# soham97/mellow

Hardware: AMD Instinct MI355X
Metric: audio-pair responses/sec (v0 167M, 2x10s clips, max_len=64, greedy) (higher is better)
Workload: dtype f32 (encoder/prefill GEMM operands split EXACTLY into 3 bf16 terms, 6 bf16 MFMA products per fp32 product, f32 accumulate: fp32-accurate, parity suite green; mel included, the STFT is an fp32 FFT; attentions and decode on exact fp32 MFMA / VALU)

## Files before the change

mellow_amd/csrc/encoder.hip:

```cpp
#include <cstdlib>

#include "common.h"
#include "kernels.h"

namespace mellow {

__global__ void reflect_pad_kernel(const float* __restrict__ wav, int64_t n, float* __restrict__ out, int64_t plen,
                                   int pad) {
    const int c = blockIdx.y;
    const float* src = wav + (int64_t)c * n;
    float* dst = out + (int64_t)c * plen;
    for (int64_t i = (int64_t)blockIdx.x * blockDim.x + threadIdx.x; i < plen; i += (int64_t)gridDim.x * blockDim.x) {
        int64_t j = i - pad;
        if (j < 0) j = -j;
        if (j >= n) j = 2 * (n - 1) - j;
        if (j < 0) j = 0;
        if (j >= n) j = n - 1;
        dst[i] = src[j];
    }
}
void launch_reflect_pad(const float* wav, int n_clips, int64_t n_samples, float* out, int64_t padded_len, int pad,
                        hipStream_t s) {
    hipLaunchKernelGGL(reflect_pad_kernel, dim3(512, n_clips), dim3(256), 0, s, wav, n_samples, out, padded_len, pad);
}
// ... 403 lines not shown
    }
}
void launch_rmsnorm_apb(const float* in, void* out_apb, int M, int C, const float* w, float eps, hipStream_t s, void* out_scales) {
    const size_t lds = (size_t)32 * (C + 4) * sizeof(float);
    set_max_dynamic_lds(reinterpret_cast<const void*>(&rmsnorm_apb_kernel<false>), 96 * 1024);
    set_max_dynamic_lds(reinterpret_cast<const void*>(&rmsnorm_apb_kernel<true>), 96 * 1024);
    if (out_scales) hipLaunchKernelGGL(rmsnorm_apb_kernel<true>, dim3((M + 31) / 32), dim3(256), lds, s, in, reinterpret_cast<i32x4*>(out_apb), (int64_t)M, C, w, eps, reinterpret_cast<uint8_t*>(out_scales));
    else hipLaunchKernelGGL(rmsnorm_apb_kernel<false>, dim3((M + 31) / 32), dim3(256), lds, s, in, reinterpret_cast<i32x4*>(out_apb), (int64_t)M, C, w, eps, (uint8_t*)nullptr);
}
void launch_rmsnorm(const float* in, float* out, int M, int C, const float* w, float eps, hipStream_t s) {
    hipLaunchKernelGGL(rmsnorm_kernel, dim3((M + 3) / 4), dim3(256), 0, s, in, out, (int64_t)M, C, w, eps);
}

__device__ __forceinline__ void wa_ld4(const float* base, int64_t elem, bool in16, float (&o)[4]) {
    if (in16) {
        typedef unsigned u32x2_ __attribute__((ext_vector_type(2)));
        const u32x2_ r = *reinterpret_cast<const u32x2_*>(reinterpret_cast<const uint16_t*>(base) + elem);
        o[0] = __uint_as_float(r[0] << 16); o[1] = __uint_as_float(r[0] & 0xffff0000u); o[2] = __uint_as_float(r[1] << 16); o[3] = __uint_as_float(r[1] & 0xffff0000u);
    } else {
        const float4 r = *reinterpret_cast<const float4*>(base + elem);
        o[0] = r.x; o[1] = r.y; o[2] = r.z; o[3] = r.w;
    }
}
template <bool IN16>
__global__ __launch_bounds__(256) void window_attention_mfma_kernel(const float* __restrict__ qkv, float* __restrict__ out,
                                                                    int C, int nH, const float* __restrict__ bias_exp,
                                                                    const float* __restrict__ mask, int nW,
                                                                    int64_t n_tiles, i32x4* __restrict__ out_apb) {
    __shared__ __attribute__((aligned(16))) float Vs[4][64 * 24];
    const int lane = threadIdx.x & 63, wave = threadIdx.x >> 6;
    const int64_t tile = (int64_t)blockIdx.x * 4 + wave;
    const bool active = tile < n_tiles;
    const int64_t win = active ? tile / nH : 0;
    const int hd = active ? (int)(tile % nH) : 0;
    const int h = lane >> 5, ml = lane & 31;
    const float scale = 0.20412414523193150818f;
    float kf[2][12], qf[2][12];
#pragma unroll
    for (int t = 0; t < 2; ++t) {
        const int64_t row = (win * 64 + t * 32 + ml) * (3 * C) + hd * 24 + 12 * h;
#pragma unroll
        for (int v = 0; v < 3; ++v) {
            float q4[4], k4[4];
            wa_ld4(qkv, row + v * 4, IN16, q4);
            wa_ld4(qkv, row + C + v * 4, IN16, k4);
#pragma unroll
            for (int j = 0; j < 4; ++j) { qf[t][4 * v + j] = q4[j] * scale; kf[t][4 * v + j] = k4[j]; }
        }
    }
    {
        const int64_t vrow = (win * 64 + lane) * (3 * C) + 2 * C + hd * 24;
#pragma unroll
        for (int v = 0; v < 6; ++v) {
            float v4[4];
            wa_ld4(qkv, vrow + v * 4, IN16, v4);
            *reinterpret_cast<float4*>(&Vs[wave][lane * 24 + v * 4]) = make_float4(v4[0], v4[1], v4[2], v4[3]);
        }
    }
    f32x16 S[2][2];
#pragma unroll
    for (int kt = 0; kt < 2; ++kt)
#pragma unroll
        for (int qt = 0; qt < 2; ++qt) {
#pragma unroll
            for (int r = 0; r < 16; ++r) S[kt][qt][r] = 0.f;
#pragma unroll
            for (int s_ = 0; s_ < 12; ++s_) S[kt][qt] = __builtin_amdgcn_mfma_f32_32x32x2f32(kf[kt][s_], qf[qt][s_], S[kt][qt], 0, 0, 0);
        }
    float inv[2];
#pragma unroll
    for (int qt = 0; qt < 2; ++qt) {
        const int qi = qt * 32 + ml;
        const float* brow = bias_exp + ((int64_t)hd * 64 + qi) * 64;
        const float* mrow = mask ? mask + ((win % nW) * 64 + qi) * 64 : nullptr;
        float mx = -INFINITY;
#pragma unroll
        for (int kt = 0; kt < 2; ++kt)
#pragma unroll
            for (int g4 = 0; g4 < 4; ++g4) {
                const int k0 = kt * 32 + 8 * g4 + 4 * h;
                const float4 b4 = *reinterpret_cast<const float4*>(brow + k0);
                float add[4] = {b4.x, b4.y, b4.z, b4.w};
                if (mrow) {
                    const float4 m4 = *reinterpret_cast<const float4*>(mrow + k0);
                    S[kt][qt][4 * g4 + 0] = (S[kt][qt][4 * g4 + 0] + add[0]) + m4.x;
                    S[kt][qt][4 * g4 + 1] = (S[kt][qt][4 * g4 + 1] + add[1]) + m4.y;
                    S[kt][qt][4 * g4 + 2] = (S[kt][qt][4 * g4 + 2] + add[2]) + m4.z;
                    S[kt][qt][4 * g4 + 3] = (S[kt][qt][4 * g4 + 3] + add[3]) + m4.w;
                } else {
#pragma unroll
                    for (int j = 0; j < 4; ++j) S[kt][qt][4 * g4 + j] += add[j];
                }
#pragma unroll
                for (int j = 0; j < 4; ++j) mx = fmaxf(mx, S[kt][qt][4 * g4 + j]);
            }
        mx = half_max(mx);
        float sum = 0.f;
#pragma unroll
        for (int kt = 0; kt < 2; ++kt)
#pragma unroll
            for (int r = 0; r < 16; ++r) {
                const float pv = __builtin_amdgcn_exp2f((S[kt][qt][r] - mx) * 1.44269504088896340736f);
                S[kt][qt][r] = pv;
                sum += pv;
            }
        inv[qt] = 1.0f / half_sum(sum);
    }
    __syncthreads();
    f32x16 O[2];
#pragma unroll
    for (int qt = 0; qt < 2; ++qt)
#pragma unroll
        for (int r = 0; r < 16; ++r) O[qt][r] = 0.f;
    const float* Vc = Vs[wave];
#pragma unroll
    for (int kt = 0; kt < 2; ++kt)
#pragma unroll
        for (int r = 0; r < 16; ++r) {
            const int key = kt * 32 + (r & 3) + 8 * (r >> 2) + 4 * h;
            const float a = ml < 24 ? Vc[key * 24 + ml] : 0.f;
            O[0] = __builtin_amdgcn_mfma_f32_32x32x2f32(a, S[kt][0][r], O[0], 0, 0, 0);
            O[1] = __builtin_amdgcn_mfma_f32_32x32x2f32(a, S[kt][1][r], O[1], 0, 0, 0);
        }
    if (active && out_apb) {
        const int KT = C >> 4;
#pragma unroll
        for (int qt = 0; qt < 2; ++qt) {
            const int64_t m = win * 64 + qt * 32 + ml;
            float X[4], Y[4], Z[4], w[8];
#pragma unroll
            for (int j = 0; j < 4; ++j) { X[j] = O[qt][j] * inv[qt]; Y[j] = O[qt][4 + j] * inv[qt]; Z[j] = O[qt][8 + j] * inv[qt]; }
            apb_store_quads(out_apb, m, hd * 3, KT, X, Y, h);
#pragma unroll
            for (int j = 0; j < 4; ++j) {
                auto r = __builtin_amdgcn_permlane32_swap(__float_as_uint(Z[j]), __float_as_uint(Z[j]), false, false);
                w[j] = __uint_as_float(r[0]);
                w[4 + j] = __uint_as_float(r[1]);
            }
            if (h == 0) apb_store8(out_apb, m, hd * 3 + 2, KT, w);
        }
    } else if (active) {
#pragma unroll
        for (int qt = 0; qt < 2; ++qt) {
            float* dst = out + (win * 64 + qt * 32 + ml) * C + hd * 24;
#pragma unroll
            for (int g4 = 0; g4 < 3; ++g4) {
                const int d = 8 * g4 + 4 * h;
                *reinterpret_cast<float4*>(dst + d) = make_float4(O[qt][4 * g4] * inv[qt], O[qt][4 * g4 + 1] * inv[qt],
                                                                  O[qt][4 * g4 + 2] * inv[qt], O[qt][4 * g4 + 3] * inv[qt]);
            }
        }
    }
}
void launch_window_attention(const float* qkv, float* out, int M, int C, int nH, const float* bias_exp,
                             const float* mask, int nW, hipStream_t s, void* out_apb, bool qkv16) {
    const int64_t n_tiles = (int64_t)(M / 64) * nH;
    if (qkv16) {
        hipLaunchKernelGGL(window_attention_mfma_kernel<true>, dim3((unsigned)((n_tiles + 3) / 4)), dim3(256), 0, s, qkv, out, C, nH,
                           bias_exp, mask, nW, n_tiles, reinterpret_cast<i32x4*>(out_apb));
        return;
    }
    hipLaunchKernelGGL(window_attention_mfma_kernel<false>, dim3((unsigned)((n_tiles + 3) / 4)), dim3(256), 0, s, qkv, out, C, nH,
                       bias_exp, mask, nW, n_tiles, reinterpret_cast<i32x4*>(out_apb));
}

__global__ __launch_bounds__(256) void tail_latent_im2col_kernel(const float* __restrict__ y, float* __restrict__ latent,
                                                                 int64_t latent_stride, float* __restrict__ a_ts) {
    const int clip = blockIdx.x;
    const float* yc = y + (int64_t)clip * 64 * 768;
    for (int ch = threadIdx.x; ch < 768; ch += 256) {
        float sacc = 0.f;
        for (int cf = 0; cf < 2; ++cf)
            for (int tt = 0; tt < 32; ++tt) {
                const int tok = ((tt >> 3) * 2 + cf) * 8 + (tt & 7);
                sacc += yc[tok * 768 + ch];
            }
        latent[(int64_t)clip * latent_stride + ch] = sacc * (1.0f / 64.0f);
    }
    float4* dst = reinterpret_cast<float4*>(a_ts + (int64_t)clip * 32 * 4608);
    for (int i = threadIdx.x; i < 32 * 6 * 192; i += 256) {
        const int c4 = i % 192;
        const int seg = (i / 192) % 6;
        const int tt = i / (192 * 6);
        const int cf = seg / 3, dt = seg % 3;
        const int ts = tt + dt - 1;
        float4 v = make_float4(0.f, 0.f, 0.f, 0.f);
// ... 179 lines not shown
```

mellow_amd/csrc/engine.cpp:

```cpp
#include "engine_internal.h"

static thread_local std::string g_err;
int fail(const char* fmt, ...) {
    char buf[1024];
    va_list ap;
    va_start(ap, fmt);
    vsnprintf(buf, sizeof(buf), fmt, ap);
    va_end(ap);
    g_err = buf;
    return 1;
}
int ensure(mellow_engine* e, mellow_engine::Buf& b, size_t floats) {
    if (b.cap >= floats) return 0;
    if (b.p) HIPCHK(hipFree(b.p));
    b.p = nullptr;
    b.cap = 0;
    HIPCHK(hipMalloc(&b.p, floats * sizeof(float)));
    b.cap = floats;
    return 0;
}
int dev_alloc(mellow_engine* e, float** out, size_t floats) {
    const size_t bytes = (floats * sizeof(float) + 4095) / 4096 * 4096;
    if (!e->arena) {
        const size_t want = (size_t)(e->opt.arena_mb < 0 ? 0 : e->opt.arena_mb) << 20;
// ... 310 lines not shown
            HIPCHK(hipStreamCreateWithFlags(&st, hipStreamNonBlocking));
            int rc = streams_overlap(e, e->stream, st, &ok);
            for (int k = 1; k < h && ok && !rc; ++k) rc = streams_overlap(e, e->stream2[k - 1], st, &ok);
            if (rc) { hipStreamDestroy(st); return rc; }
            if (ok) e->stream2[h - 1] = st; else hipStreamDestroy(st);
        }
        if (!ok) {
            e->prefill_parts_want = e->prefill_parts;
            e->prefill_parts = e->prefill_parts_ok = h;
            e->streams_probed = true;
            break;
        }
    }
    return 0;
}
struct OptDesc { const char* key; const char* dflt; bool answers; const char* what; };
static const OptDesc kOptions[] = {
    {"prefill_split", "2", false, "f32x3: parts of the split LM prefill (1..4); bit-identical for every value"},
    {"prefill_fuse_norm", "1", true, "f32x3: norm-free LM prefill (GEMM epilogues emit split output + RMS partials); 0 = a normalisation launch per GEMM input"},
    {"decode_fuse", "1", true, "down projection of layer l fused with q/k/v of layer l + 1 through the load-time product W'Wd; 0 = five launches per layer"},
    {"decode_fuse_max_rb", "1", true, "largest number of 32-row blocks that runs the fused down + q/k/v launch on fp32 weights"},
    {"splitk", "8", true, "f32x3 encoder: largest split count of the split-K launches (0 = never split; a summation order)"},
    {"enc_apb", "0x1CC", false, "f32x3 encoder: Swin stages whose producers hand over pre-split (bit st, 4 + st, 8 + st); bit-identical"},
    {"graph", "1", false, "decode steps as hipGraph replays (0 = eager launches)"},
    {"fp8_decode", "1", true, "fp8 mode: e4m3 weights in the decode kernels"},
    {"fp8_prefill", "1", true, "fp8 mode: e4m3 GEMMs in encoder + LM prefill"},
    {"fp8_decode_act", "1", true, "fp8 mode: e4m3 activations in the decode GEMM kernels (fp8 matrix pipe)"},
    {"fp8_kv16", "1", true, "fp8 mode: bf16 shadow of the K/V pages for the decode step"},
    {"fp8_attn_bf16", "1", true, "fp8 mode: q / k / v stored once as bf16 (LM: bf16 K/V pages + bf16-once prefill attention; Swin: bf16 q/k/v rows into the exact window attention); 0 = fp32 q/k/v, the 3-way split attention"},
    {"decode_x3", "7", true, "f32x3: mask of decode GEMM launches on the bf16 pipe (1 lm_head, 2 gate/up, 4 fused down + q/k/v)"},
    {"decode_x3_min_rb", "2", true, "f32x3: fewest 32-row blocks at which the layer launches take their f32x3 forms"},
    {"x3_stft", "1", true, "f32x3: STFT / mel GEMMs on the split kernel (0 = exact fp32 kernel)"},
    {"stft_fft", "1", true, "f32x3: STFT as a 1024-point FFT when the checkpoint's conv weights are the windowed DFT basis"},
    {"x3_apb", "1", true, "f32x3 LM prefill: producers hand over pre-split, GEMMs staged by LDS-DMA (0 = register-staged kernel on fp32 activations)"},
    {"x3_attn", "1", true, "f32x3: prefill attention on exact bf16 splits (0 = exact fp32 MFMA kernel)"},
    {"x3w", "1", false, "f32x3: K = 96 GEMMs on the weight-stationary persistent kernel; bit-identical"},
    {"row_migration", "1", false, "reference-semantics loop, B > 32: rows still running are packed into the lowest 32-row blocks; tokens unchanged"},
    {"arena_mb", "3400", false, "size of the weight arena in MiB (before the first tensor is loaded)"},
};
static const OptDesc* find_opt(const char* key) {
    for (const auto& o : kOptions)
        if (!strcmp(o.key, key)) return &o;
    return nullptr;
}
static long opt_val(const mellow_engine* e, const char* key) {
    auto it = e->opt.given.find(key);
    return strtol(it != e->opt.given.end() ? it->second.c_str() : find_opt(key)->dflt, nullptr, 0);
}
int apply_options(mellow_engine* e) {
    const int mode = e->opt.mode;
    e->prefill_parts = (int)opt_val(e, "prefill_split");
    e->opt.prefill_fuse_norm = opt_val(e, "prefill_fuse_norm") != 0;
    e->opt.decode_fuse = opt_val(e, "decode_fuse") != 0;
    e->opt.dec_fuse_max_rb = (int)opt_val(e, "decode_fuse_max_rb");
    e->opt.sk_max = (int)opt_val(e, "splitk");
    e->opt.enc_apb_stages = (int)opt_val(e, "enc_apb");
    e->use_graph = opt_val(e, "graph") != 0;
    e->opt.x3_stft = opt_val(e, "x3_stft") != 0;
    e->opt.stft_fft = opt_val(e, "stft_fft") != 0 && e->opt.x3_stft;
    e->opt.x3_apb = opt_val(e, "x3_apb") != 0;
    e->opt.x3_attn = opt_val(e, "x3_attn") != 0;
    e->opt.x3w = opt_val(e, "x3w") != 0;
    e->opt.row_migration = opt_val(e, "row_migration") != 0;
    e->opt.arena_mb = (int)opt_val(e, "arena_mb");
    e->opt.fp8 = mode == MELLOW_PRECISION_FP8;
    e->opt.fp8_decode = e->opt.fp8 && opt_val(e, "fp8_decode") != 0;
    e->opt.fp8_decode_act = e->opt.fp8_decode && opt_val(e, "fp8_decode_act") != 0;
    e->opt.fp8_prefill = opt_val(e, "fp8_prefill") != 0;
    e->opt.fp8_attn_bf16 = opt_val(e, "fp8_attn_bf16") != 0;
    e->opt.kv16 = e->opt.fp8_decode && opt_val(e, "fp8_kv16") != 0;
    e->opt.f32x3_terms = mode == MELLOW_PRECISION_F32X3 ? 6 : 0;
    e->opt.dec_x3 = mode == MELLOW_PRECISION_F32X3 ? ((int)opt_val(e, "decode_x3") & DEC_X3_ALL) : 0;
    e->opt.dec_x3_min_rb = (int)opt_val(e, "decode_x3_min_rb") < 1 ? 1 : (int)opt_val(e, "decode_x3_min_rb");
    return 0;
}

extern "C" {

int mellow_engine_set_option(mellow_engine_t* e, const char* key, const char* value) {
// ... 135 lines not shown
```

mellow_amd/csrc/engine_encoder.cpp:

```cpp
#include "engine_internal.h"

static void with_splitk(mellow_engine* e, GemmArgs& g) {
    if (!e->sk_enable || e->opt.sk_max < 2 || !e->sk_ws.p) return;
    g.sk_ws = e->sk_ws.p;
    g.sk_tiles = 256;
    g.sk_max = e->opt.sk_max;
}
int run_gemm(mellow_engine* e, const GemmArgs& a) {
    const bool x3_stft = e->opt.x3_stft;
    if (e->opt.f32x3_terms && a.K % 16 == 0 &&
        ((a.a_mode == A_PLAIN && (a.epi == EPI_LINEAR || a.epi == EPI_SWIGLU || a.epi == EPI_QKV_ROPE || a.epi == EPI_QKV_ROPE_AT)) || (x3_stft && a.K >= 192))) {
        auto it = e->w.bf_w.find(a.Wp);
        if (it != e->w.bf_w.end()) {
            GemmArgs g = a;
            g.W8 = reinterpret_cast<const uint8_t*>(it->second);
            with_splitk(e, g);
            ProfScope ps(e, PF_GEMM, gemm_flops(a), 0.0);
            ps.r.M = a.M; ps.r.N = a.Nw; ps.r.K = a.K; ps.r.epi = a.epi + 200;
            launch_gemm_bf16x3_fused(g, e->stream);
            return 0;
        }
    }
    if (e->opt.fp8 && e->opt.fp8_prefill && a.a_mode == A_PLAIN && (a.epi == EPI_LINEAR || a.epi == EPI_SWIGLU || a.epi == EPI_QKV_ROPE)) {
        auto it = e->w.fp8_w.find(a.Wp);
// ... 104 lines not shown
    CHK(ensure(e, e->QKV, (size_t)M0 * 288));
    CHK(ensure(e, e->H, (size_t)M0 * 384));
    {
        ProfScope ps(e, PF_MISC, 0, (double)M0 * 96 * 4);
        launch_fold_patch_embed(e->logmel.p, n, frames, n_crops, crop_hop, crop_len, e->w.pe_w, e->w.pe_b, e->w.pe_nw, e->w.pe_nb,
                                e->X0.p, s);
    }
    CHK(tap(e, "patch", e->X0.p, M0 * 96));
    float *x = e->X0.p, *x2 = e->X1.p, *t = e->T.p;
    for (int st = 0; st < 4; ++st) {
        const int C = 96 << st, R = 64 >> st, N = R * R, nH = kHeads[st];
        const int nW = R > kWin ? (R / kWin) * (R / kWin) : 1;
        const int M1 = nv * N;
        for (int b = 0; b < kDepths[st]; ++b) {
            const SwinBlockW& w = e->w.blocks[st][b];
            const bool shifted = (b % 2 == 1) && R > kWin;
            const int32_t* map = R > kWin ? e->w.win_map[st][shifted ? 1 : 0] : nullptr;
            const bool amx = e->opt.fp8 && e->opt.fp8_prefill && e->opt.x3_apb && e->w.fp8_w.count(w.qkv.p) && e->w.fp8_w.count(w.fc1.p) && e->w.fp8_w.count(w.fc2.p);
            const bool have_pb = e->opt.f32x3_terms && e->w.bf_w.count(w.qkv.p) && e->w.bf_w.count(w.fc1.p) && e->w.bf_w.count(w.fc2.p);
            const bool apb_h = amx || (have_pb && ((e->opt.enc_apb_stages >> st) & 1));
            const bool apb = apb_h || (have_pb && ((e->opt.enc_apb_stages >> (8 + st)) & 1));
            const size_t M1p = (size_t)rup(M1, 128);
            char *a3s = nullptr, *h3s = nullptr;
            if (apb) {
                CHK(ensure(e, e->enc_a3, (M1p * C * 6 + 3) / 4));
                if (apb_h) CHK(ensure(e, e->enc_h3, (M1p * 4 * C * 6 + 3) / 4));
                if (amx) {
                    a3s = reinterpret_cast<char*>(e->enc_a3.p) + M1p * rup(C, 64);
                    h3s = reinterpret_cast<char*>(e->enc_h3.p) + M1p * rup(4 * C, 64);
                }
                { ProfScope ps(e, PF_NORM, 0, 2.5 * M1 * C * 4); launch_layernorm_apb(x, e->enc_a3.p, M1, C, w.n1w, w.n1b, map, N, s, a3s); }
                {
                    GemmArgs g = lin(nullptr, C, M1, w.qkv, e->QKV.p, 3 * C, w.qkv_b);
                    g.c16 = (amx && e->opt.fp8_attn_bf16) ? 1 : 0;
                    CHK(run_gemm_apb(e, g, e->enc_a3.p, s, a3s));
                }
            } else {
                { ProfScope ps(e, PF_NORM, 0, 2.0 * M1 * C * 4); launch_layernorm(x, t, M1, C, w.n1w, w.n1b, map, N, s); }
                CHK(run_gemm(e, lin(t, C, M1, w.qkv, e->QKV.p, 3 * C, w.qkv_b)));
            }
            const bool apb_proj = apb && !amx && ((e->opt.enc_apb_stages >> (4 + st)) & 1) && e->w.bf_w.count(w.proj.p);
            {
                ProfScope ps(e, PF_WINDOW_ATTN, 4.0 * 64 * 64 * 24 * (double)(M1 / 64) * nH, 4.0 * M1 * C * 4);
                launch_window_attention(e->QKV.p, t, M1, C, nH, w.bias_exp, shifted ? w.mask : nullptr, nW, s, apb_proj ? e->enc_a3.p : nullptr, amx && e->opt.fp8_attn_bf16);
            }
            {
                GemmArgs g = lin(t, C, M1, w.proj, x, C, w.proj_b);
                g.resid = x; g.ldr = C; g.crow_map = map; g.rows_in = N; g.rows_out = N;
                if (apb_proj) CHK(run_gemm_apb(e, g, e->enc_a3.p, s));
                else CHK(run_gemm(e, g));
            }
            if (apb) {
                { ProfScope ps(e, PF_NORM, 0, 2.5 * M1 * C * 4); launch_layernorm_apb(x, e->enc_a3.p, M1, C, w.n2w, w.n2b, nullptr, N, s, a3s); }
                {
                    GemmArgs g = lin(nullptr, C, M1, w.fc1, apb_h ? nullptr : e->H.p, 4 * C, w.fc1_b);
                    g.act = ACT_GELU; g.C3 = apb_h ? e->enc_h3.p : nullptr;
                    if (amx) { g.c3_fmt = 1; g.C3s = reinterpret_cast<uint8_t*>(h3s); g.c3_kt64 = rup(4 * C, 64) / 64; }
                    CHK(run_gemm_apb(e, g, e->enc_a3.p, s, a3s));
                }
                {
                    GemmArgs g = lin(apb_h ? nullptr : e->H.p, 4 * C, M1, w.fc2, x, C, w.fc2_b);
                    g.resid = x; g.ldr = C;
                    if (apb_h) CHK(run_gemm_apb(e, g, e->enc_h3.p, s, h3s));
                    else CHK(run_gemm(e, g));
                }
            } else {
                { ProfScope ps(e, PF_NORM, 0, 2.0 * M1 * C * 4); launch_layernorm(x, t, M1, C, w.n2w, w.n2b, nullptr, N, s); }
                {
                    GemmArgs g = lin(t, C, M1, w.fc1, e->H.p, 4 * C, w.fc1_b);
                    g.act = ACT_GELU;
                    CHK(run_gemm(e, g));
                }
// ... 167 lines not shown
```

mellow_amd/csrc/engine_internal.h:

```cpp
#pragma once
#include <hip/hip_runtime.h>

#include <array>
#include <chrono>
#include <cmath>
#include <cstdarg>
#include <cstdio>
#include <cstdlib>
#include <cstring>
#include <map>
#include <unordered_map>
#include <string>
#include <thread>
#include <type_traits>
#include <utility>
#include <vector>

#include "../../include/mellow_hip.h"
#include "kernels.h"

using namespace mellow;

int fail(const char* fmt, ...);
struct mellow_engine;
// ... 30 lines not shown
    std::vector<char> data;
    std::vector<int64_t> shape;
    int dtype = 0;
    int64_t numel() const {
        int64_t n = 1;
        for (auto d : shape) n *= d;
        return n;
    }
    const float* f() const { return reinterpret_cast<const float*>(data.data()); }
};

struct Packed {
    float* p = nullptr;
    int N = 0, K = 0, NP = 0, KP = 0;
    int Nw = 0;
};

struct SwinBlockW {
    float *n1w, *n1b, *n2w, *n2b;
    Packed qkv, proj, fc1, fc2;
    float *qkv_b, *proj_b, *fc1_b, *fc2_b;
    float* bias_exp;
    float* mask;
};
struct MergeW {
    float *nw, *nb;
    Packed red;
};
struct DecW {
    const float *p, *scale;
};
struct LMLayerW {
    Packed qkv, o, gateup, down;
    Packed qkv_f, gateup_f;
    float* o16 = nullptr;
    float* gu16n = nullptr;
    float* gu16 = nullptr;
    float* qkv2 = nullptr;
    float *q2h8 = nullptr, *q2h_sc = nullptr;
    float *qkv8 = nullptr, *qkv_sc = nullptr, *o8 = nullptr, *o_sc = nullptr, *gu8 = nullptr, *gu_sc = nullptr, *dn8 = nullptr,
          *dn_sc = nullptr;
    float *in_ln, *post_ln;
    DecW qkv_w() const { return qkv8 ? DecW{qkv8, qkv_sc} : DecW{qkv_f.p, nullptr}; }
    DecW o_w() const { return o8 ? DecW{o8, o_sc} : DecW{o16, nullptr}; }
    DecW gateup_w() const { return gu8 ? DecW{gu8, gu_sc} : DecW{gu16, nullptr}; }
    DecW down_w() const { return dn8 ? DecW{dn8, dn_sc} : DecW{down.p, nullptr}; }
// ... 45 lines not shown
        float* p = nullptr;
        size_t cap = 0;
        Buf() = default; Buf(const Buf&) = delete; Buf& operator=(const Buf&) = delete;
        Buf(Buf&& o) noexcept : p(o.p), cap(o.cap) { o.p = nullptr; o.cap = 0; }
        Buf& operator=(Buf&& o) noexcept { std::swap(p, o.p); std::swap(cap, o.cap); return *this; }
        LOCAL ~Buf() { if (p) (void)hipFree(p); }
    };
    struct LOCAL Options {
        std::map<std::string, std::string> given;
        int mode = MELLOW_PRECISION_F32X3;
        bool x3_stft = true, stft_fft = true, x3_apb = true, x3_attn = true, x3w = true, row_migration = true, decode_fuse = true;
        int arena_mb = 3400;
        bool kv16 = false;
        bool fp8 = false;
        bool fp8_decode = false;
        bool fp8_decode_act = false;
        bool fp8_attn_bf16 = true;
        bool fp8_prefill = true;
        int dec_x3_min_rb = 2;
        int dec_x3 = 0;
        int f32x3_terms = 0;
        bool prefill_fuse_norm = true;
        int enc_apb_stages = 0x1CC;
        int sk_max = 8;
        int dec_fuse_max_rb = 1;
    };
    struct Fp8W { uint8_t* w8; float* scale; };
    struct LOCAL Weights {
        Packed dft, mel;
        float *fft_win = nullptr, *fft_tw1 = nullptr, *fft_tw2 = nullptr;
        float *bn_alpha = nullptr, *bn_beta = nullptr;
        float *pe_w = nullptr, *pe_b = nullptr, *pe_nw = nullptr, *pe_nb = nullptr;
        std::vector<SwinBlockW> blocks[4];
        MergeW merge[3];
        int32_t* win_map[4][2] = {{nullptr}};
        float *fn_w = nullptr, *fn_b = nullptr;
        Packed tscam, c2l, lin1, lin2;
        float *tscam_b = nullptr, *c2l_b = nullptr, *pln_w = nullptr, *pln_b = nullptr;
        int32_t* emb_row_map = nullptr;
        float* embed = nullptr;
        Packed lm_head;
        std::vector<LMLayerW> layers;
        float* final_norm = nullptr;
        float *rope_cos = nullptr, *rope_sin = nullptr;
        float *head8 = nullptr, *head_sc = nullptr;
        DecW head_w() const { return head8 ? DecW{head8, head_sc} : DecW{lm_head.p, nullptr}; }
// ... 206 lines not shown
```

mellow_amd/csrc/engine_weights.cpp:

```cpp
#include "engine_internal.h"

static const HostTensor* get(mellow_engine* e, const std::string& k) {
    auto it = e->host.find(k);
    return it == e->host.end() ? nullptr : &it->second;
}
static int expect_shape(const HostTensor* t, const std::string& k, std::initializer_list<int64_t> shp) {
    if (!t) return fail("missing key in state_dict: %s", k.c_str());
    if (t->dtype != MELLOW_F32) return fail("%s: expected float32", k.c_str());
    if (t->shape.size() != shp.size())
        return fail("size mismatch for %s: rank %d in the checkpoint, %d expected", k.c_str(), (int)t->shape.size(), (int)shp.size());
    size_t i = 0;
    for (auto d : shp) {
        if (t->shape[i] != d)
            return fail("size mismatch for %s: dimension %d is %lld in the checkpoint, %lld expected", k.c_str(), (int)i,
                        (long long)t->shape[i], (long long)d);
        ++i;
    }
    return 0;
}
static int up_vec(mellow_engine* e, const std::string& k, int64_t n, float** out, int64_t pad_to = 0) {
    const HostTensor* t = get(e, k);
    CHK(expect_shape(t, k, {n}));
    return upload(e, out, t->f(), (size_t)n, (size_t)pad_to);
}
// ... 151 lines not shown
        CHK(upload(e, &e->w.pe_w, get(e, k)->f(), 96 * 16));
        CHK(up_vec(e, E + "patch_embed.proj.bias", 96, &e->w.pe_b));
        CHK(up_vec(e, E + "patch_embed.norm.weight", 96, &e->w.pe_nw));
        CHK(up_vec(e, E + "patch_embed.norm.bias", 96, &e->w.pe_nb));
    }
    for (int s = 0; s < 4; ++s) {
        const int C = 96 << s, nH = kHeads[s], R = 64 >> s, nW = (R / kWin) * (R / kWin);
        for (int sh = 0; sh < 2; ++sh) {
            if (R <= kWin) continue;
            std::vector<int32_t> m((size_t)R * R);
            window_map_host(R, sh ? kWin / 2 : 0, m.data());
            float* d = nullptr;
            CHK(upload(e, &d, reinterpret_cast<const float*>(m.data()), m.size()));
            e->w.win_map[s][sh] = reinterpret_cast<int32_t*>(d);
        }
        for (int b = 0; b < kDepths[s]; ++b) {
            const std::string p = E + "layers." + std::to_string(s) + ".blocks." + std::to_string(b) + ".";
            SwinBlockW w{};
            CHK(up_vec(e, p + "norm1.weight", C, &w.n1w));
            CHK(up_vec(e, p + "norm1.bias", C, &w.n1b));
            CHK(up_vec(e, p + "norm2.weight", C, &w.n2w));
            CHK(up_vec(e, p + "norm2.bias", C, &w.n2b));
            CHK(pack_key(e, p + "attn.qkv.weight", 3 * C, C, &w.qkv));
            CHK(pack_key(e, p + "attn.proj.weight", C, C, &w.proj));
            CHK(pack_key(e, p + "mlp.fc1.weight", 4 * C, C, &w.fc1));
            CHK(pack_key(e, p + "mlp.fc2.weight", C, 4 * C, &w.fc2));
            CHK(up_vec(e, p + "attn.qkv.bias", 3 * C, &w.qkv_b, w.qkv.NP));
            CHK(up_vec(e, p + "attn.proj.bias", C, &w.proj_b, w.proj.NP));
            CHK(up_vec(e, p + "mlp.fc1.bias", 4 * C, &w.fc1_b, w.fc1.NP));
            CHK(up_vec(e, p + "mlp.fc2.bias", C, &w.fc2_b, w.fc2.NP));
            const HostTensor *tb = get(e, p + "attn.relative_position_bias_table"), *ix = get(e, p + "attn.relative_position_index");
            CHK(expect_shape(tb, p + "attn.relative_position_bias_table", {225, nH}));
            if (ix->numel() != 64 * 64) return fail("size mismatch for %sattn.relative_position_index", p.c_str());
            std::vector<float> be((size_t)nH * 4096);
            for (int i = 0; i < 4096; ++i) {
                int64_t id;
                if (ix->dtype == MELLOW_I64) id = reinterpret_cast<const int64_t*>(ix->data.data())[i];
                else id = reinterpret_cast<const int32_t*>(ix->data.data())[i];
                if (id < 0 || id >= 225) return fail("relative_position_index out of range");
                for (int h = 0; h < nH; ++h) be[(size_t)h * 4096 + i] = tb->f()[id * nH + h];
            }
            CHK(upload(e, &w.bias_exp, be.data(), be.size()));
            w.mask = nullptr;
            if ((b % 2 == 1) && R > kWin) {
                const std::string km = p + "attn_mask";
                CHK(expect_shape(get(e, km), km, {nW, 64, 64}));
// ... 160 lines not shown
```

mellow_amd/csrc/kernels.h:

```cpp
#pragma once
#include <hip/hip_runtime.h>
#include <stdint.h>

namespace mellow {

void launch_pack_weight(const float* w, int N, int K, int64_t ldw, float* out, int NP, int KP, hipStream_t s);
void launch_pack_weight_pairs(const float* w0, const float* w1, int N, int K, int64_t ldw, float* out, int NP,
                              int KP, hipStream_t s);

enum { ACT_NONE = 0, ACT_GELU = 1, ACT_SIGMOID = 2 };
enum { EPI_LINEAR = 0, EPI_POWER = 1, EPI_LOGMEL = 2, EPI_SWIGLU = 3, EPI_QKV_ROPE = 4, EPI_LSE = 5, EPI_QKV_ROPE_AT = 6 };
enum { A_PLAIN = 0, A_FRAMES = 1 };

struct GemmArgs {
    const float* A = nullptr;
    int64_t lda = 0;
    int M = 0;
    int K = 0;
    int a_mode = A_PLAIN;
    int fpc = 1;
    int64_t clip_stride = 0;
    int hop = 0;
    const float* Wp = nullptr;
    int Nw = 0;
// ... 242 lines not shown
void set_gemm_debug_buffer(uint64_t* p);

void launch_resample(const float* x, int n_clips, int64_t n_in, const float* wT, int orig, int nw, int klen, int width,
                     float* out, int64_t n_out, hipStream_t s);
void launch_reflect_pad(const float* wav, int n_clips, int64_t n_samples, float* out, int64_t padded_len, int pad,
                        hipStream_t s);
void launch_fold_patch_embed(const float* logmel_bn, int n_src, int src_frames, int n_crops, int crop_hop,
                             int crop_len, const float* conv_w, const float* conv_b, const float* ln_w,
                             const float* ln_b, float* x0, hipStream_t s);

void launch_layernorm(const float* in, float* out, int M, int C, const float* w, const float* b,
                      const int32_t* row_map, int ntok, hipStream_t s);
void launch_merge_layernorm(const float* in, float* out, int n, int R, int C, const float* w, const float* b,
                            hipStream_t s);
void launch_stft_fft_power(const float* wpad, int fpc, int64_t clip_stride, int hop, int M, const float* win, const float* tw1,
                           const float* tw2, float* power, hipStream_t s);
void launch_rmsnorm(const float* in, float* out, int M, int C, const float* w, float eps, hipStream_t s);
void launch_layernorm_apb(const float* in, void* out_apb, int M, int C, const float* w, const float* b, const int32_t* row_map,
                          int ntok, hipStream_t s, void* out_scales = nullptr);
void launch_rmsnorm_apb(const float* in, void* out_apb, int M, int C, const float* w, float eps, hipStream_t s, void* out_scales = nullptr);

void launch_window_attention(const float* qkv, float* out, int M, int C, int nH, const float* bias_exp,
                             const float* mask, int nW, hipStream_t s, void* out_apb = nullptr, bool qkv16 = false);

void launch_tail_latent_im2col(const float* y, int n, float* latent, int64_t latent_stride, float* a_ts,
                               hipStream_t s);
void launch_crop_average(const float* in, int n, int n_crops, int64_t len, int64_t in_stride, float* out,
                         int64_t out_stride, hipStream_t s);
void launch_gelu(const float* in, float* out, int64_t n, hipStream_t s);
void launch_prefix_assemble(const float* proj33, const float* embed, const int32_t* ids, int B, int text_len,
                            int sep_id, int vocab, float* prefix, unsigned long long* bad_id_word, hipStream_t s);
void launch_prefix_assemble_q(const float* proj33, const float* embed, const int32_t* ids, int B, int Q, int text_len, int P,
                              int sep_id, int vocab, float* head, float* tail, unsigned long long* bad_id_word, hipStream_t s);
void launch_gather_rows(const float* table, int width, const int32_t* ids, int n, int n_rows, float* out, hipStream_t s);
void launch_gather_span(const float* in, int B, int T, int from_pos, int n, float* out, hipStream_t s);
void launch_clear_page_slots(float* cache, int64_t pages, int Tmax, int t0, int t1, hipStream_t s, bool pages16 = false);
void launch_downsample33(const float* proj33, int n, float* out, hipStream_t s);

void launch_prefill_attention(const float* q, const float* k_cache, const float* v_cache, float* o, void* o_apb, int B, int T,
                              int Tmax, bool x3, hipStream_t s, void* o_scales = nullptr, bool bf16_once = false, bool pages16 = false);
void launch_prefill_attention_past(const float* q, const float* k_cache, const float* v_cache, float* o, void* o_apb, int B, int T,
                                   int Tmax, int q0, bool x3, hipStream_t s);
void launch_lse_merge(const float2* part_ms, const int32_t* part_arg, int64_t ld, int groups, int rows, const int32_t* targets,
                      const float* tgt_logit, int vocab, float* out_logprob, int32_t* out_argmax, float* out_lse, float* out_max,
                      unsigned long long* bad_word, hipStream_t s);
void launch_score_build_input(const float* prefix, const float* embed, const int32_t* cand_ids, const int32_t* cand_len, int K,
// ... 7 lines not shown
```

Before: 459.6.

## Fuse Swin qkv GEMM with window attention for early encoder stages

Adds a kernel that computes the per-head q/k/v projection with split-bf16 MFMA for each 64-token window and feeds the result straight into the existing window attention tile. This avoids writing and re-reading the full QKV tensor for stages 0 (enabled by default via a bitmask option). Per-head weights are pre-packed at load time and staged in LDS. The cost is a persistent-style grid with heavier register and LDS use per workgroup, which may reduce occupancy compared with the separate GEMM.

```diff
diff --git a/mellow_amd/csrc/encoder.hip b/mellow_amd/csrc/encoder.hip
--- a/mellow_amd/csrc/encoder.hip
+++ b/mellow_amd/csrc/encoder.hip
@@ -449,6 +449,105 @@
         o[0] = r.x; o[1] = r.y; o[2] = r.z; o[3] = r.w;
     }
 }
+__device__ __forceinline__ void window_attention_tile(const float (&kf)[2][12], const float (&qf)[2][12], const float* Vc, float* __restrict__ out,
+                                                      int C, int64_t win, int hd, bool active, const float* __restrict__ bias_exp,
+                                                      const float* __restrict__ mask, int nW, i32x4* __restrict__ out_apb) {
+    const int lane = threadIdx.x & 63;
+    const int h = lane >> 5, ml = lane & 31;
+    f32x16 S[2][2];
+#pragma unroll
+    for (int kt = 0; kt < 2; ++kt)
+#pragma unroll
+        for (int qt = 0; qt < 2; ++qt) {
+#pragma unroll
+            for (int r = 0; r < 16; ++r) S[kt][qt][r] = 0.f;
+#pragma unroll
+            for (int s_ = 0; s_ < 12; ++s_) S[kt][qt] = __builtin_amdgcn_mfma_f32_32x32x2f32(kf[kt][s_], qf[qt][s_], S[kt][qt], 0, 0, 0);
+        }
+    float inv[2];
+#pragma unroll
+    for (int qt = 0; qt < 2; ++qt) {
+        const int qi = qt * 32 + ml;
+        const float* brow = bias_exp + ((int64_t)hd * 64 + qi) * 64;
+        const float* mrow = mask ? mask + ((win % nW) * 64 + qi) * 64 : nullptr;
+        float mx = -INFINITY;
+#pragma unroll
+        for (int kt = 0; kt < 2; ++kt)
+#pragma unroll
+            for (int g4 = 0; g4 < 4; ++g4) {
+                const int k0 = kt * 32 + 8 * g4 + 4 * h;
+                const float4 b4 = *reinterpret_cast<const float4*>(brow + k0);
+                float add[4] = {b4.x, b4.y, b4.z, b4.w};
+                if (mrow) {
+                    const float4 m4 = *reinterpret_cast<const float4*>(mrow + k0);
+                    S[kt][qt][4 * g4 + 0] = (S[kt][qt][4 * g4 + 0] + add[0]) + m4.x;
+                    S[kt][qt][4 * g4 + 1] = (S[kt][qt][4 * g4 + 1] + add[1]) + m4.y;
+                    S[kt][qt][4 * g4 + 2] = (S[kt][qt][4 * g4 + 2] + add[2]) + m4.z;
+                    S[kt][qt][4 * g4 + 3] = (S[kt][qt][4 * g4 + 3] + add[3]) + m4.w;
+                } else {
+#pragma unroll
+                    for (int j = 0; j < 4; ++j) S[kt][qt][4 * g4 + j] += add[j];
+                }
+#pragma unroll
+                for (int j = 0; j < 4; ++j) mx = fmaxf(mx, S[kt][qt][4 * g4 + j]);
+            }
+        mx = half_max(mx);
+        float sum = 0.f;
+#pragma unroll
+        for (int kt = 0; kt < 2; ++kt)
+#pragma unroll
+            for (int r = 0; r < 16; ++r) {
+                const float pv = __builtin_amdgcn_exp2f((S[kt][qt][r] - mx) * 1.44269504088896340736f);
+                S[kt][qt][r] = pv;
+                sum += pv;
+            }
+        inv[qt] = 1.0f / half_sum(sum);
+    }
+    __syncthreads();
+    f32x16 O[2];
+#pragma unroll
+    for (int qt = 0; qt < 2; ++qt)
+#pragma unroll
+        for (int r = 0; r < 16; ++r) O[qt][r] = 0.f;
+#pragma unroll
+    for (int kt = 0; kt < 2; ++kt)
+#pragma unroll
+        for (int r = 0; r < 16; ++r) {
+            const int key = kt * 32 + (r & 3) + 8 * (r >> 2) + 4 * h;
+            const float a = ml < 24 ? Vc[key * 24 + ml] : 0.f;
+            O[0] = __builtin_amdgcn_mfma_f32_32x32x2f32(a, S[kt][0][r], O[0], 0, 0, 0);
+            O[1] = __builtin_amdgcn_mfma_f32_32x32x2f32(a, S[kt][1][r], O[1], 0, 0, 0);
+        }
+    if (active && out_apb) {
+        const int KT = C >> 4;
+#pragma unroll
+        for (int qt = 0; qt < 2; ++qt) {
+            const int64_t m = win * 64 + qt * 32 + ml;
+            float X[4], Y[4], Z[4], w[8];
+#pragma unroll
+            for (int j = 0; j < 4; ++j) { X[j] = O[qt][j] * inv[qt]; Y[j] = O[qt][4 + j] * inv[qt]; Z[j] = O[qt][8 + j] * inv[qt]; }
+            apb_store_quads(out_apb, m, hd * 3, KT, X, Y, h);
+#pragma unroll
+            for (int j = 0; j < 4; ++j) {
+                auto r = __builtin_amdgcn_permlane32_swap(__float_as_uint(Z[j]), __float_as_uint(Z[j]), false, false);
+                w[j] = __uint_as_float(r[0]);
+                w[4 + j] = __uint_as_float(r[1]);
+            }
+            if (h == 0) apb_store8(out_apb, m, hd * 3 + 2, KT, w);
+        }
+    } else if (active) {
+#pragma unroll
+        for (int qt = 0; qt < 2; ++qt) {
+            float* dst = out + (win * 64 + qt * 32 + ml) * C + hd * 24;
+#pragma unroll
+            for (int g4 = 0; g4 < 3; ++g4) {
+                const int d = 8 * g4 + 4 * h;
+                *reinterpret_cast<float4*>(dst + d) = make_float4(O[qt][4 * g4] * inv[qt], O[qt][4 * g4 + 1] * inv[qt],
+                                                                  O[qt][4 * g4 + 2] * inv[qt], O[qt][4 * g4 + 3] * inv[qt]);
+            }
+        }
+    }
+}
 template <bool IN16>
 __global__ __launch_bounds__(256) void window_attention_mfma_kernel(const float* __restrict__ qkv, float* __restrict__ out,
                                                                     int C, int nH, const float* __restrict__ bias_exp,
@@ -484,100 +583,7 @@
             *reinterpret_cast<float4*>(&Vs[wave][lane * 24 + v * 4]) = make_float4(v4[0], v4[1], v4[2], v4[3]);
         }
     }
-    f32x16 S[2][2];
-#pragma unroll
-    for (int kt = 0; kt < 2; ++kt)
-#pragma unroll
-        for (int qt = 0; qt < 2; ++qt) {
-#pragma unroll
-            for (int r = 0; r < 16; ++r) S[kt][qt][r] = 0.f;
-#pragma unroll
-            for (int s_ = 0; s_ < 12; ++s_) S[kt][qt] = __builtin_amdgcn_mfma_f32_32x32x2f32(kf[kt][s_], qf[qt][s_], S[kt][qt], 0, 0, 0);
-        }
-    float inv[2];
-#pragma unroll
-    for (int qt = 0; qt < 2; ++qt) {
-        const int qi = qt * 32 + ml;
-        const float* brow = bias_exp + ((int64_t)hd * 64 + qi) * 64;
-        const float* mrow = mask ? mask + ((win % nW) * 64 + qi) * 64 : nullptr;
-        float mx = -INFINITY;
-#pragma unroll
-        for (int kt = 0; kt < 2; ++kt)
-#pragma unroll
-            for (int g4 = 0; g4 < 4; ++g4) {
-                const int k0 = kt * 32 + 8 * g4 + 4 * h;
-                const float4 b4 = *reinterpret_cast<const float4*>(brow + k0);
-                float add[4] = {b4.x, b4.y, b4.z, b4.w};
-                if (mrow) {
-                    const float4 m4 = *reinterpret_cast<const float4*>(mrow + k0);
-                    S[kt][qt][4 * g4 + 0] = (S[kt][qt][4 * g4 + 0] + add[0]) + m4.x;
-                    S[kt][qt][4 * g4 + 1] = (S[kt][qt][4 * g4 + 1] + add[1]) + m4.y;
-                    S[kt][qt][4 * g4 + 2] = (S[kt][qt][4 * g4 + 2] + add[2]) + m4.z;
-                    S[kt][qt][4 * g4 + 3] = (S[kt][qt][4 * g4 + 3] + add[3]) + m4.w;
-                } else {
-#pragma unroll
-                    for (int j = 0; j < 4; ++j) S[kt][qt][4 * g4 + j] += add[j];
-                }
-#pragma unroll
-                for (int j = 0; j < 4; ++j) mx = fmaxf(mx, S[kt][qt][4 * g4 + j]);
-            }
-        mx = half_max(mx);
-        float sum = 0.f;
-#pragma unroll
-        for (int kt = 0; kt < 2; ++kt)
-#pragma unroll
-            for (int r = 0; r < 16; ++r) {
-                const float pv = __builtin_amdgcn_exp2f((S[kt][qt][r] - mx) * 1.44269504088896340736f);
-                S[kt][qt][r] = pv;
-                sum += pv;
-            }
-        inv[qt] = 1.0f / half_sum(sum);
-    }
-    __syncthreads();
-    f32x16 O[2];
-#pragma unroll
-    for (int qt = 0; qt < 2; ++qt)
-#pragma unroll
-        for (int r = 0; r < 16; ++r) O[qt][r] = 0.f;
-    const float* Vc = Vs[wave];
-#pragma unroll
-    for (int kt = 0; kt < 2; ++kt)
-#pragma unroll
-        for (int r = 0; r < 16; ++r) {
-            const int key = kt * 32 + (r & 3) + 8 * (r >> 2) + 4 * h;
-            const float a = ml < 24 ? Vc[key * 24 + ml] : 0.f;
-            O[0] = __builtin_amdgcn_mfma_f32_32x32x2f32(a, S[kt][0][r], O[0], 0, 0, 0);
-            O[1] = __builtin_amdgcn_mfma_f32_32x32x2f32(a, S[kt][1][r], O[1], 0, 0, 0);
-        }
-    if (active && out_apb) {
-        const int KT = C >> 4;
-#pragma unroll
-        for (int qt = 0; qt < 2; ++qt) {
-            const int64_t m = win * 64 + qt * 32 + ml;
-            float X[4], Y[4], Z[4], w[8];
-#pragma unroll
-            for (int j = 0; j < 4; ++j) { X[j] = O[qt][j] * inv[qt]; Y[j] = O[qt][4 + j] * inv[qt]; Z[j] = O[qt][8 + j] * inv[qt]; }
-            apb_store_quads(out_apb, m, hd * 3, KT, X, Y, h);
-#pragma unroll
-            for (int j = 0; j < 4; ++j) {
-                auto r = __builtin_amdgcn_permlane32_swap(__float_as_uint(Z[j]), __float_as_uint(Z[j]), false, false);
-                w[j] = __uint_as_float(r[0]);
-                w[4 + j] = __uint_as_float(r[1]);
-            }
-            if (h == 0) apb_store8(out_apb, m, hd * 3 + 2, KT, w);
-        }
-    } else if (active) {
-#pragma unroll
-        for (int qt = 0; qt < 2; ++qt) {
-            float* dst = out + (win * 64 + qt * 32 + ml) * C + hd * 24;
-#pragma unroll
-            for (int g4 = 0; g4 < 3; ++g4) {
-                const int d = 8 * g4 + 4 * h;
-                *reinterpret_cast<float4*>(dst + d) = make_float4(O[qt][4 * g4] * inv[qt], O[qt][4 * g4 + 1] * inv[qt],
-                                                                  O[qt][4 * g4 + 2] * inv[qt], O[qt][4 * g4 + 3] * inv[qt]);
-            }
-        }
-    }
+    window_attention_tile(kf, qf, Vs[wave], out, C, win, hd, active, bias_exp, mask, nW, out_apb);
 }
 void launch_window_attention(const float* qkv, float* out, int M, int C, int nH, const float* bias_exp,
                              const float* mask, int nW, hipStream_t s, void* out_apb, bool qkv16) {
@@ -589,6 +595,152 @@
     }
     hipLaunchKernelGGL(window_attention_mfma_kernel<false>, dim3((unsigned)((n_tiles + 3) / 4)), dim3(256), 0, s, qkv, out, C, nH,
                        bias_exp, mask, nW, n_tiles, reinterpret_cast<i32x4*>(out_apb));
+}
+
+__global__ __launch_bounds__(256) void pack_qkv_heads_kernel(const i32x4* __restrict__ PB, int C, int nH, i32x4* __restrict__ out) {
+    const int KT = C >> 4;
+    const int total = nH * KT * 9 * 64;
+    for (int i = blockIdx.x * 256 + threadIdx.x; i < total; i += gridDim.x * 256) {
+        const int lane = i & 63, f = (i >> 6) % 9, kt = (i / (9 * 64)) % KT, hd = i / (9 * 64 * KT);
+        const int sec = f / 3, pc = f % 3;
+        const int j = lane & 31, kh = lane >> 5;
+        const int hr = (j >> 2) & 1, rr = (j & 3) + 4 * (j >> 3);
+        i32x4 v = {0, 0, 0, 0};
+        if (rr < 12) {
+            const int n = sec * C + hd * 24 + 12 * hr + rr;
+            v = PB[(((int64_t)(n >> 5) * KT + kt) * 3 + pc) * 64 + (n & 31) + 32 * kh];
+        }
+        out[i] = v;
+    }
+}
+void launch_pack_qkv_heads(const void* PB, int C, int nH, void* out, hipStream_t s) {
+    const int total = nH * (C >> 4) * 9 * 64;
+    hipLaunchKernelGGL(pack_qkv_heads_kernel, dim3((unsigned)((total + 255) / 256)), dim3(256), 0, s, reinterpret_cast<const i32x4*>(PB), C, nH,
+                       reinterpret_cast<i32x4*>(out));
+}
+template <int KT, bool APB_IN>
+__device__ __forceinline__ void swin_qkv_attn_tile(const void* __restrict__ a_in, const i32x4* wp, const float* __restrict__ qkv_b, float* Vw,
+                                                   float* __restrict__ out, int64_t win, int hd, bool active, const float* __restrict__ bias_exp,
+                                                   const float* __restrict__ mask, int nW, i32x4* __restrict__ out_apb) {
+    constexpr int C = KT * 16;
+    const int lane = threadIdx.x & 63;
+    const int h = lane >> 5, ml = lane & 31;
+    f32x16 acc[3][2];
+#pragma unroll
+    for (int s_ = 0; s_ < 3; ++s_)
+#pragma unroll
+        for (int t = 0; t < 2; ++t)
+#pragma unroll
+            for (int r = 0; r < 16; ++r) acc[s_][t][r] = 0.f;
+    const i32x4* ap = reinterpret_cast<const i32x4*>(a_in) + ((win >> 1) * KT * 12 + 2 * (win & 1)) * 64 + lane;
+    const float* ar = reinterpret_cast<const float*>(a_in) + (win * 64 + ml) * C + 8 * h;
+#define QA_BF(W, A, ACC) ACC = __builtin_amdgcn_mfma_f32_32x32x16_bf16(__builtin_bit_cast(bf16x8, W), __builtin_bit_cast(bf16x8, A), ACC, 0, 0, 0);
+#define QA_TERM(PW, PA)                                                                  \
+    _Pragma("unroll") for (int s_ = 0; s_ < 3; ++s_) {                                   \
+        QA_BF(w[s_][PW], a[0][PA], acc[s_][0])                                           \
+        QA_BF(w[s_][PW], a[1][PA], acc[s_][1])                                           \
+    }
+    i32x4 ra[3][6];
+    auto load_a = [&](int kt, i32x4 (&r)[6]) {
+#pragma unroll
+        for (int t = 0; t < 2; ++t) {
+            if (APB_IN) {
+#pragma unroll
+                for (int pc = 0; pc < 3; ++pc) r[t * 3 + pc] = ap[(kt * 12 + pc * 4 + t) * 64];
+            } else {
+                r[t * 2] = *reinterpret_cast<const i32x4*>(ar + t * 32 * C + kt * 16);
+                r[t * 2 + 1] = *reinterpret_cast<const i32x4*>(ar + t * 32 * C + kt * 16 + 4);
+            }
+        }
+    };
+    load_a(0, ra[0]);
+    load_a(1, ra[1]);
+#pragma unroll
+    for (int kt = 0; kt < KT; ++kt) {
+        i32x4 a[2][3], w[3][3];
+        if (kt + 2 < KT) load_a(kt + 2, ra[(kt + 2) % 3]);
+#pragma unroll
+        for (int t = 0; t < 2; ++t) {
+            if (APB_IN) {
+#pragma unroll
+                for (int pc = 0; pc < 3; ++pc) a[t][pc] = ra[kt % 3][t * 3 + pc];
+            } else {
+                const i32x4 lo = ra[kt % 3][t * 2], hi = ra[kt % 3][t * 2 + 1];
+                const float v[8] = {__int_as_float(lo[0]), __int_as_float(lo[1]), __int_as_float(lo[2]), __int_as_float(lo[3]),
+                                    __int_as_float(hi[0]), __int_as_float(hi[1]), __int_as_float(hi[2]), __int_as_float(hi[3])};
+                split8(v, a[t][0], a[t][1], a[t][2]);
+            }
+        }
+#pragma unroll
+        for (int s_ = 0; s_ < 3; ++s_)
+#pragma unroll
+            for (int pc = 0; pc < 3; ++pc) w[s_][pc] = wp[(kt * 9 + s_ * 3 + pc) * 64];
+        QA_TERM(2, 0) QA_TERM(0, 2) QA_TERM(1, 1) QA_TERM(1, 0) QA_TERM(0, 1) QA_TERM(0, 0)
+        __builtin_amdgcn_sched_barrier(0);
+    }
+#undef QA_TERM
+#undef QA_BF
+    const float scale = 0.20412414523193150818f;
+    float kf[2][12], qf[2][12];
+    const float* bp = qkv_b + hd * 24 + 12 * h;
+#pragma unroll
+    for (int v = 0; v < 3; ++v) {
+        const float4 bq = *reinterpret_cast<const float4*>(bp + 4 * v), bk = *reinterpret_cast<const float4*>(bp + C + 4 * v),
+                     bv = *reinterpret_cast<const float4*>(bp + 2 * C + 4 * v);
+        const float q4[4] = {bq.x, bq.y, bq.z, bq.w}, k4[4] = {bk.x, bk.y, bk.z, bk.w}, v4[4] = {bv.x, bv.y, bv.z, bv.w};
+#pragma unroll
+        for (int t = 0; t < 2; ++t) {
+            float vv[4];
+#pragma unroll
+            for (int j = 0; j < 4; ++j) {
+                const float q = acc[0][t][4 * v + j] + q4[j];
+                qf[t][4 * v + j] = q * scale;
+                kf[t][4 * v + j] = acc[1][t][4 * v + j] + k4[j];
+                vv[j] = acc[2][t][4 * v + j] + v4[j];
+            }
+            *reinterpret_cast<float4*>(&Vw[(t * 32 + ml) * 24 + 12 * h + 4 * v]) = make_float4(vv[0], vv[1], vv[2], vv[3]);
+        }
+    }
+    window_attention_tile(kf, qf, Vw, out, C, win, hd, active, bias_exp, mask, nW, out_apb);
+}
+template <int KT, bool APB_IN, int NWV>
+__global__ __launch_bounds__(NWV * 64, 8 / NWV) void swin_qkv_attn_kernel(const void* __restrict__ a_in, const i32x4* __restrict__ pbh,
+                                                                          const float* __restrict__ qkv_b, float* __restrict__ out, int nH,
+                                                                          const float* __restrict__ bias_exp, const float* __restrict__ mask,
+                                                                          int nW, int64_t n_win, i32x4* __restrict__ out_apb) {
+    extern __shared__ __attribute__((aligned(16))) i32x4 smem_qa[];
+    i32x4* Ws = smem_qa;
+    float* Vs = reinterpret_cast<float*>(smem_qa + KT * 9 * 64);
+    const int lane = threadIdx.x & 63, wave = threadIdx.x >> 6;
+    const int b = (int)blockIdx.x;
+    const int hd = (b >> 3) % nH, g = (b & 7) + 8 * (b / (8 * nH)), G = (int)gridDim.x / nH;
+    for (int i = threadIdx.x; i < KT * 9 * 64; i += NWV * 64) Ws[i] = pbh[(int64_t)hd * KT * 9 * 64 + i];
+    __syncthreads();
+    for (int64_t win0 = (int64_t)g * NWV; win0 < n_win; win0 += (int64_t)G * NWV) {
+        const bool active = win0 + wave < n_win;
+        swin_qkv_attn_tile<KT, APB_IN>(a_in, Ws + lane, qkv_b, Vs + wave * (64 * 24), out, active ? win0 + wave : 0, hd, active, bias_exp, mask, nW, out_apb);
+    }
+}
+bool launch_swin_qkv_attn(const void* a, bool a_apb, const void* pbh, const float* qkv_b, float* out, int M, int C, int nH, const float* bias_exp,
+                          const float* mask, int nW, hipStream_t s, void* out_apb) {
+    if ((C != 96 && C != 192) || nH * 24 != C || M % 64) return false;
+    const int64_t n_win = M / 64;
+    const i32x4* w = reinterpret_cast<const i32x4*>(pbh);
+    i32x4* o3 = reinterpret_cast<i32x4*>(out_apb);
+    const int nwv = C == 96 ? 4 : 8, n_wg = C == 96 ? 512 : 256;
+    int64_t G = (n_win + nwv - 1) / nwv < n_wg / nH ? (n_win + nwv - 1) / nwv : n_wg / nH;
+    G = (G + 7) / 8 * 8;
+    const dim3 grid((unsigned)(G * nH)), block(nwv * 64);
+    const size_t lds = (size_t)(C / 16) * 9 * 1024 + (size_t)nwv * 64 * 24 * sizeof(float);
+#define QA_LAUNCH(KT, APB, NWV)                                                                                         \
+    {                                                                                                                   \
+        set_max_dynamic_lds(reinterpret_cast<const void*>(&swin_qkv_attn_kernel<KT, APB, NWV>), lds);                   \
+        hipLaunchKernelGGL((swin_qkv_attn_kernel<KT, APB, NWV>), grid, block, lds, s, a, w, qkv_b, out, nH, bias_exp, mask, nW, n_win, o3); \
+    }
+    if (C == 96) { if (a_apb) QA_LAUNCH(6, true, 4) else QA_LAUNCH(6, false, 4) }
+    else { if (a_apb) QA_LAUNCH(12, true, 8) else QA_LAUNCH(12, false, 8) }
+#undef QA_LAUNCH
+    return true;
 }
 
 __global__ __launch_bounds__(256) void tail_latent_im2col_kernel(const float* __restrict__ y, float* __restrict__ latent,
diff --git a/mellow_amd/csrc/engine.cpp b/mellow_amd/csrc/engine.cpp
--- a/mellow_amd/csrc/engine.cpp
+++ b/mellow_amd/csrc/engine.cpp
@@ -356,6 +356,7 @@
     {"decode_fuse_max_rb", "1", true, "largest number of 32-row blocks that runs the fused down + q/k/v launch on fp32 weights"},
     {"splitk", "8", true, "f32x3 encoder: largest split count of the split-K launches (0 = never split; a summation order)"},
     {"enc_apb", "0x1CC", false, "f32x3 encoder: Swin stages whose producers hand over pre-split (bit st, 4 + st, 8 + st); bit-identical"},
+    {"enc_qkv_attn", "0x1", false, "f32x3 encoder: Swin stages (bit st, stages 0-1) whose qkv GEMM and window attention run as one launch, no QKV tensor; bit-identical"},
     {"graph", "1", false, "decode steps as hipGraph replays (0 = eager launches)"},
     {"fp8_decode", "1", true, "fp8 mode: e4m3 weights in the decode kernels"},
     {"fp8_prefill", "1", true, "fp8 mode: e4m3 GEMMs in encoder + LM prefill"},
@@ -389,6 +390,7 @@
     e->opt.dec_fuse_max_rb = (int)opt_val(e, "decode_fuse_max_rb");
     e->opt.sk_max = (int)opt_val(e, "splitk");
     e->opt.enc_apb_stages = (int)opt_val(e, "enc_apb");
+    e->opt.enc_qkv_attn = (int)opt_val(e, "enc_qkv_attn");
     e->use_graph = opt_val(e, "graph") != 0;
     e->opt.x3_stft = opt_val(e, "x3_stft") != 0;
     e->opt.stft_fft = opt_val(e, "stft_fft") != 0 && e->opt.x3_stft;
diff --git a/mellow_amd/csrc/engine_encoder.cpp b/mellow_amd/csrc/engine_encoder.cpp
--- a/mellow_amd/csrc/engine_encoder.cpp
+++ b/mellow_amd/csrc/engine_encoder.cpp
@@ -150,6 +150,9 @@
             const bool apb = apb_h || (have_pb && ((e->opt.enc_apb_stages >> (8 + st)) & 1));
             const size_t M1p = (size_t)rup(M1, 128);
             char *a3s = nullptr, *h3s = nullptr;
+            const bool apb_proj = apb && !amx && ((e->opt.enc_apb_stages >> (4 + st)) & 1) && e->w.bf_w.count(w.proj.p);
+            const bool fused_attn = st < 2 && ((e->opt.enc_qkv_attn >> st) & 1) && e->opt.f32x3_terms && !e->opt.fp8 && w.qkv_pbh &&
+                                    e->w.bf_w.count(w.qkv.p) && M1 % 64 == 0;
             if (apb) {
                 CHK(ensure(e, e->enc_a3, (M1p * C * 6 + 3) / 4));
                 if (apb_h) CHK(ensure(e, e->enc_h3, (M1p * 4 * C * 6 + 3) / 4));
@@ -157,6 +160,19 @@
                     a3s = reinterpret_cast<char*>(e->enc_a3.p) + M1p * rup(C, 64);
                     h3s = reinterpret_cast<char*>(e->enc_h3.p) + M1p * rup(4 * C, 64);
                 }
+            }
+            const void* attn3 = e->enc_a3.p;
+            if (fused_attn) {
+                attn3 = e->QKV.p;
+                if (apb) { ProfScope ps(e, PF_NORM, 0, 2.5 * M1 * C * 4); launch_layernorm_apb(x, e->enc_a3.p, M1, C, w.n1w, w.n1b, map, N, s, nullptr); }
+                else { ProfScope ps(e, PF_NORM, 0, 2.0 * M1 * C * 4); launch_layernorm(x, e->QKV.p, M1, C, w.n1w, w.n1b, map, N, s); }
+                const GemmArgs g = lin(nullptr, C, M1, w.qkv, nullptr, 3 * C, w.qkv_b);
+                ProfScope ps(e, PF_GEMM, gemm_flops(g), 0.0);
+                ps.r.M = g.M; ps.r.N = g.Nw; ps.r.K = g.K; ps.r.epi = g.epi + 600;
+                if (!launch_swin_qkv_attn(apb ? (const void*)e->enc_a3.p : (const void*)e->QKV.p, apb, w.qkv_pbh, w.qkv_b, t, M1, C, nH, w.bias_exp,
+                                          shifted ? w.mask : nullptr, nW, s, apb_proj ? e->QKV.p : nullptr))
+                    return fail("internal: no fused q/k/v + window attention kernel for C = %d", C);
+            } else if (apb) {
                 { ProfScope ps(e, PF_NORM, 0, 2.5 * M1 * C * 4); launch_layernorm_apb(x, e->enc_a3.p, M1, C, w.n1w, w.n1b, map, N, s, a3s); }
                 {
                     GemmArgs g = lin(nullptr, C, M1, w.qkv, e->QKV.p, 3 * C, w.qkv_b);
@@ -167,15 +183,14 @@
                 { ProfScope ps(e, PF_NORM, 0, 2.0 * M1 * C * 4); launch_layernorm(x, t, M1, C, w.n1w, w.n1b, map, N, s); }
                 CHK(run_gemm(e, lin(t, C, M1, w.qkv, e->QKV.p, 3 * C, w.qkv_b)));
             }
-            const bool apb_proj = apb && !amx && ((e->opt.enc_apb_stages >> (4 + st)) & 1) && e->w.bf_w.count(w.proj.p);
-            {
+            if (!fused_attn) {
                 ProfScope ps(e, PF_WINDOW_ATTN, 4.0 * 64 * 64 * 24 * (double)(M1 / 64) * nH, 4.0 * M1 * C * 4);
                 launch_window_attention(e->QKV.p, t, M1, C, nH, w.bias_exp, shifted ? w.mask : nullptr, nW, s, apb_proj ? e->enc_a3.p : nullptr, amx && e->opt.fp8_attn_bf16);
             }
             {
                 GemmArgs g = lin(t, C, M1, w.proj, x, C, w.proj_b);
                 g.resid = x; g.ldr = C; g.crow_map = map; g.rows_in = N; g.rows_out = N;
-                if (apb_proj) CHK(run_gemm_apb(e, g, e->enc_a3.p, s));
+                if (apb_proj) CHK(run_gemm_apb(e, g, attn3, s));
                 else CHK(run_gemm(e, g));
             }
             if (apb) {
diff --git a/mellow_amd/csrc/engine_internal.h b/mellow_amd/csrc/engine_internal.h
--- a/mellow_amd/csrc/engine_internal.h
+++ b/mellow_amd/csrc/engine_internal.h
@@ -76,6 +76,7 @@
     float *qkv_b, *proj_b, *fc1_b, *fc2_b;
     float* bias_exp;
     float* mask;
+    float* qkv_pbh;
 };
 struct MergeW {
     float *nw, *nb;
@@ -167,6 +168,7 @@
         int f32x3_terms = 0;
         bool prefill_fuse_norm = true;
         int enc_apb_stages = 0x1CC;
+        int enc_qkv_attn = 0x1;
         int sk_max = 8;
         int dec_fuse_max_rb = 1;
     };
diff --git a/mellow_amd/csrc/engine_weights.cpp b/mellow_amd/csrc/engine_weights.cpp
--- a/mellow_amd/csrc/engine_weights.cpp
+++ b/mellow_amd/csrc/engine_weights.cpp
@@ -197,6 +197,12 @@
             CHK(up_vec(e, p + "norm2.weight", C, &w.n2w));
             CHK(up_vec(e, p + "norm2.bias", C, &w.n2b));
             CHK(pack_key(e, p + "attn.qkv.weight", 3 * C, C, &w.qkv));
+            if (s < 2 && w.qkv.KP == C && e->w.bf_w.count(w.qkv.p)) {
+                CHK(dev_alloc(e, &w.qkv_pbh, (size_t)nH * (C / 16) * 9 * 64 * 4));
+                launch_pack_qkv_heads(e->w.bf_w[w.qkv.p], C, nH, w.qkv_pbh, e->stream);
+                HIPCHK(hipGetLastError());
+                HIPCHK(hipStreamSynchronize(e->stream));
+            }
             CHK(pack_key(e, p + "attn.proj.weight", C, C, &w.proj));
             CHK(pack_key(e, p + "mlp.fc1.weight", 4 * C, C, &w.fc1));
             CHK(pack_key(e, p + "mlp.fc2.weight", C, 4 * C, &w.fc2));
diff --git a/mellow_amd/csrc/kernels.h b/mellow_amd/csrc/kernels.h
--- a/mellow_amd/csrc/kernels.h
+++ b/mellow_amd/csrc/kernels.h
@@ -288,6 +288,9 @@
 
 void launch_window_attention(const float* qkv, float* out, int M, int C, int nH, const float* bias_exp,
                              const float* mask, int nW, hipStream_t s, void* out_apb = nullptr, bool qkv16 = false);
+void launch_pack_qkv_heads(const void* PB, int C, int nH, void* out, hipStream_t s);
+bool launch_swin_qkv_attn(const void* a, bool a_apb, const void* pbh, const float* qkv_b, float* out, int M, int C, int nH, const float* bias_exp,
+                          const float* mask, int nW, hipStream_t s, void* out_apb = nullptr);
 
 void launch_tail_latent_im2col(const float* y, int n, float* latent, int64_t latent_stride, float* a_ts,
                                hipStream_t s);
```

New measurement: 459.4, median of 2. About the same (-0.0%).
